# openai/whisper

Measured on AMD Instinct MI355X. Metric: audio-seconds transcribed per wall-second (large-v3 greedy), higher is better.
Workload: dtype f16

## Files before the change

whisper_amd/csrc/gemv.hip:

```cpp
#include "common.h"
#include "kernels.h"
#include <stdlib.h>

#ifndef WH_GEMV8_MAX_ROWS
#define WH_GEMV8_MAX_ROWS 24
#endif

namespace {

#define ISSUE_FENCE() asm volatile("" ::: "memory")

constexpr int CS = 4;

__device__ __forceinline__ float4v load_part4(const float* p) { return *(const float4v*)p; }
__device__ __forceinline__ float4v load_part4(const half_t* p) {
  const half4v h = *(const half4v*)p;
  return float4v{(float)h[0], (float)h[1], (float)h[2], (float)h[3]};
}

template <typename T> struct Pack4;
template <> struct Pack4<float> {
  static __device__ __forceinline__ void store(float* p, float a, float b, float c, float d) {
    *(float4v*)p = float4v{a, b, c, d};
  }
// ... 856 lines not shown
    }
    const bool diag = (lane >> 5) == ((lane >> 3) & 1);
#pragma unroll
    for (int rt = 0; rt < NRT; ++rt) {
      float4v acc = {0.f, 0.f, 0.f, 0.f};
      if constexpr (XW != 0) {
        half8v xt[NU];
#pragma unroll
        for (int u = 0; u < NU; ++u) xt[u] = xfrag[rt * FRAG + (kw * NU + u) * 64 + lane];
#pragma unroll
        for (int u = 0; u < NU; ++u) acc = __builtin_amdgcn_mfma_f32_16x16x32_f16(wa[u], xt[u], acc, 0, 0, 0);
      } else {
#pragma unroll
        for (int u = 0; u < NU; ++u) acc = __builtin_amdgcn_mfma_f32_16x16x32_f16(wa[u], xb[rt][u], acc, 0, 0, 0);
      }
#pragma unroll
      for (int e = 0; e < 4; ++e) {
        float z = diag ? acc[e] : 0.f;
        z += lane_xor8(z);
        float p, q; lane_swap32(z, p, q);
        acc[e] = p + q;
      }
      if (lane < 32 && (lane & 15) < 8) {
#pragma unroll
        for (int e = 0; e < 4; ++e) red[mw][rt][4 * (lane >> 4) + e][lane & 7] = acc[e];
      }
    }
  }
  WH_PROBE_AT(a, wgid, 4);
  __syncthreads();
  WH_PROBE_AT(a, wgid, 5);
#pragma unroll
  for (int j = 0; j < NOUT; ++j) {
    const int o = tid + NT * j;
    const int es = o / (NRT * 64), ert = (o >> 6) % NRT, er = (o >> 3) & 7, ej = o & 7;
    const int en = blockIdx.x * fw + es * 8 + ej;
    const bool on = o < GS * NRT * 64 && ert * 8 + er < R && es * 8 + ej < fw && en < a.N;
    if (on) {
      float v = e_bias[j];
#pragma unroll
      for (int k = 0; k < KS; ++k) v += red[es * KS + k][ert][ej][er];
      const int64_t rr = r0 + ert * 8 + er;
      const int n = en;
      switch (a.epi) {
        case whk::EPI_STORE: ((half_t*)a.y)[a.y_frag ? frag_elem(rr, n, a.N) : rr * a.y_ld + n] = (half_t)v; break;
        case whk::EPI_GELU: ((half_t*)a.y)[a.y_frag ? frag_elem(rr, n, a.N) : rr * a.y_ld + n] = (half_t)gelu_erf(v); break;
        case whk::EPI_F32: ((float*)a.y)[rr * a.y_ld + n] = v; break;
        case whk::EPI_RESID: a.resid[rr * a.resid_ld + n] = e_res[j] + v; break;
        case whk::EPI_QKV: {
          const int D = a.D;
          if (n < D) ((half_t*)a.y)[rr * a.y_ld + n] = (half_t)v;
          else {
            const int64_t pos = e_pos - e_lag[j];
            if (n < 2 * D) ((half_t*)a.kcache)[rr * a.cache_bs + pos * D + (n - D)] = (half_t)v;
            else ((half_t*)a.vcache)[rr * a.cache_bs + pos * D + (n - 2 * D)] = (half_t)v;
          }
        } break;
      }
    }
  }
  WH_PROBE_AT(a, wgid, 6);
  if (a.bump && blockIdx.x == 0 && blockIdx.y == 0 && tid == 0) atomicAdd(a.bump, a.bump_by);
  if (a.bump2 && blockIdx.x == 0 && blockIdx.y == 0 && tid == 0) atomicAdd(a.bump2, 1);
}

template <int PRO, int GS, int KS, int CSm, int XW, int NRT>
hipError_t launch_gemv8_nrt(const whk::GemvArgs& a, int fw, hipStream_t stream) {
  constexpr int WAVES = GS * KS + XW;
  static_assert(WAVES <= 16, "at most 1024 threads per workgroup");
  if (fw < 1 || fw > 8 * GS) return hipErrorInvalidValue;
  whk::g_form = WH_FORM_NAME("gemv8/%s/gs%d/ks%d/xw%d/rt%d", PRO == whk::PRO_PLAIN ? "plain" : PRO == whk::PRO_LN ? "LN" :
                             CSm == 2 ? "combine2" : CSm == 3 ? "combine3" : "combine4", GS, KS, XW, NRT);
  const int nblk = a.K / 64;
  const int nu = (nblk + KS - 1) / KS;
  dim3 grid((a.N + fw - 1) / fw, (a.R + 8 * NRT - 1) / (8 * NRT)), block(WAVES * 64);
  if constexpr (KS == 2) {
    if (nu > 10) return hipErrorInvalidValue;
    hipLaunchKernelGGL((gemv8_kernel<PRO, GS, KS, 10, CSm, XW, NRT>), grid, block, 0, stream, a, fw);
  } else {
    if (nu <= 3) hipLaunchKernelGGL((gemv8_kernel<PRO, GS, KS, 3, CSm, XW, NRT>), grid, block, 0, stream, a, fw);
    else if (nu <= 5) hipLaunchKernelGGL((gemv8_kernel<PRO, GS, KS, 5, CSm, XW, NRT>), grid, block, 0, stream, a, fw);
    else return hipErrorInvalidValue;
  }
  return hipGetLastError();
}

template <int PRO, int GS, int KS, int CSm, int XW>
hipError_t launch_gemv8_cfg(const whk::GemvArgs& a, int fw, hipStream_t stream) {
  if (a.R <= 8) return launch_gemv8_nrt<PRO, GS, KS, CSm, XW, 1>(a, fw, stream);
  if (a.R <= 16) return launch_gemv8_nrt<PRO, GS, KS, CSm, XW, 2>(a, fw, stream);
  if constexpr (GS * KS + XW < 16) {
    if (a.R > 24) return launch_gemv8_nrt<PRO, GS, KS, CSm, XW, 6>(a, fw, stream);
  }
  return launch_gemv8_nrt<PRO, GS, KS, CSm, XW, 3>(a, fw, stream);
}

static int gemv8_fw(int N, int gs) {
  static int ncu = 256;
  int fw = (N + ncu - 1) / ncu;
  if (fw > 8 * gs) fw = 8 * gs;
  if (fw < 4) fw = N < 8 ? N : 8 < 8 * gs ? 8 : 8 * gs;
  return fw;
}

static int gemv8_slots(int N, int pro) {
  const int ngroups = (N + 7) / 8;
  if (pro == whk::PRO_LN) return ngroups >= 600 ? 3 : ngroups >= 400 ? 2 : 1;
  return 1;
}

template <int PRO, int CSm>
hipError_t launch_gemv8_pro(const whk::GemvArgs& a, hipStream_t stream) {
  const int nblk = a.K / 64, gs = gemv8_slots(a.N, PRO), fw = gemv8_fw(a.N, gs);
  if constexpr (PRO == whk::PRO_PLAIN) {
    if (nblk > 20) {
      whk::GemvArgs b = a;
      b.w_ordered = !WH_DEV_FLAG("WH_GEMV8_W_OPERAND_ORDER");
      return launch_gemv8_cfg<PRO, 1, 16, CSm, 0>(b, fw, stream);
    }
    return launch_gemv8_cfg<PRO, 1, 4, CSm, 0>(a, fw, stream);
  } else {
    if constexpr (PRO == whk::PRO_LN) {
      if (gs == 3 && a.R > 8 && !WH_DEV_FLAG("WH_GEMV8_LN3_KS4")) {
        if (a.R <= 16) return launch_gemv8_nrt<PRO, 3, 2, CSm, 8, 2>(a, fw, stream);
        return launch_gemv8_nrt<PRO, 3, 2, CSm, 8, 3>(a, fw, stream);
      }
      if (gs == 3) return launch_gemv8_cfg<PRO, 3, 4, CSm, 4>(a, fw, stream);
      if (gs == 2) return launch_gemv8_cfg<PRO, 2, 4, CSm, 8>(a, fw, stream);
    }
    return launch_gemv8_cfg<PRO, 1, 4, CSm, 8>(a, fw, stream);
  }
}

bool gemv8_applies(const whk::GemvArgs& a) {
  if (WH_DEV_FLAG("WH_GEMV_DOT2")) return false;
  if (a.variant != 0 || a.R < 1 || a.R > 96 || a.K % 64 != 0) return false;
  const int nblk = a.K / 64;
  if (nblk > 20 && (a.pro != whk::PRO_PLAIN || (nblk + 15) / 16 > 5)) return false;
  if (a.epi == whk::EPI_F32 && a.N > 16384) return false;
  if ((int64_t)a.N * a.K >= (1ll << 31)) return false;
  switch (a.pro) {
    case whk::PRO_PLAIN: return a.x_ld % 8 == 0 && (int64_t)a.R * a.x_ld < (1ll << 30);
    case whk::PRO_LN: return a.ln_folded && a.xf_ld % 4 == 0 && (int64_t)a.R * a.xf_ld < (1ll << 29);
    case whk::PRO_COMBINE:
      return a.K == a.H * 64 && a.H <= 20 && a.splits >= 2 && a.splits <= 4 && (int64_t)a.R * a.H * a.splits * 64 < (1ll << 29);
  }
  return false;
}

hipError_t launch_gemv8(const whk::GemvArgs& a, hipStream_t stream) {
  if (a.pro == whk::PRO_PLAIN) return launch_gemv8_pro<whk::PRO_PLAIN, 1>(a, stream);
  if (a.pro == whk::PRO_LN) return launch_gemv8_pro<whk::PRO_LN, 1>(a, stream);
  if (a.pro == whk::PRO_COMBINE && a.splits == 2) return launch_gemv8_pro<whk::PRO_COMBINE, 2>(a, stream);
  if (a.pro == whk::PRO_COMBINE && a.splits == 3) return launch_gemv8_pro<whk::PRO_COMBINE, 3>(a, stream);
  if (a.pro == whk::PRO_COMBINE && a.splits == 4) return launch_gemv8_pro<whk::PRO_COMBINE, 4>(a, stream);
  return hipErrorInvalidValue;
}

template <int NFT>
__global__ __launch_bounds__(1024) void gemv_rows48_kernel(whk::GemvArgs a) {
  extern __shared__ __attribute__((aligned(16))) char smem[];
  pin_kernargs(a);
  constexpr int WAVES = 16, RT = 48, KSP = WAVES / NFT, J = 5, NU = (40 + KSP - 1) / KSP;
  const int K = a.K, nks = K / 32;
  half_t* xs = (half_t*)smem;
  float* red = (float*)smem;
  const int tid = threadIdx.x, lane = tid & 63;
  const int wave = __builtin_amdgcn_readfirstlane(tid >> 6);
  const int ft = wave % NFT, ksp = wave / NFT;
  const int i16 = lane & 15, g4 = lane >> 4;
  const int n0 = blockIdx.x * (NFT * 16);
  const int R = a.R;

  float4v v[3][J];
#pragma unroll
  for (int i = 0; i < 3; ++i) {
    const int r = wave + WAVES * i;
    const float* src = a.xf + (int64_t)(r < R ? r : 0) * a.xf_ld;
#pragma unroll
    for (int j = 0; j < J; ++j) {
      int k = (j * 64 + lane) * 4; if (k > K - 4) k = K - 4;
      v[i][j] = *(const float4v*)(src + k);
    }
  }
  ISSUE_FENCE();
  half8v w[NU];
  {
    int n = n0 + ft * 16 + i16; if (n > a.N - 1) n = a.N - 1;
    const half_t* base = (const half_t*)a.W + (int64_t)n * K + g4 * 8;
#pragma unroll
    for (int u = 0; u < NU; ++u) {
      int st = ksp + KSP * u; if (st > nks - 1) st = nks - 1;
      w[u] = __builtin_nontemporal_load((const half8v*)(base + st * 32));
    }
  }
  ISSUE_FENCE();
  int e_pos = 0;
  if (a.epi == whk::EPI_QKV) e_pos = load_agent_int(a.d_pos);
  float e_bias[(NFT * 768 + 1023) / 1024];
#pragma unroll
  for (int q = 0; q < (NFT * 768 + 1023) / 1024; ++q) {
    const int o = tid + q * 1024;
    int n = n0 + ((o >> 8) / 3) * 16 + (o & 15); if (n > a.N - 1) n = a.N - 1;
    e_bias[q] = a.bias ? a.bias[n] : 0.f;
  }

  {
    const float invK = 1.0f / (float)K;
#pragma unroll
    for (int i = 0; i < 3; ++i) {
      const int r = wave + WAVES * i;
      float sum = 0.f;
#pragma unroll
      for (int j = 0; j < J; ++j) {
        const float t = (v[i][j][0] + v[i][j][1]) + (v[i][j][2] + v[i][j][3]);
        sum += ((j * 64 + lane) * 4 < K) ? t : 0.f;
      }
      const float mean = wave_sum(sum) * invK;
      float ss = 0.f;
#pragma unroll
      for (int j = 0; j < J; ++j) {
        if ((j * 64 + lane) * 4 < K) {
#pragma unroll
          for (int e = 0; e < 4; ++e) { const float d = v[i][j][e] - mean; ss = __builtin_fmaf(d, d, ss); }
        }
      }
      const float rstd = r < R ? rsqrtf(wave_sum(ss) * invK + 1e-5f) : 0.f;
      half_t* xr = xs + (size_t)r * K;
#pragma unroll
      for (int j = 0; j < J; ++j) {
        const int k = (j * 64 + lane) * 4;
        if (k < K)
          Pack4<half_t>::store(xr + ((((k >> 3) ^ (r & 15)) << 3) | (k & 7)), (v[i][j][0] - mean) * rstd,
                               (v[i][j][1] - mean) * rstd, (v[i][j][2] - mean) * rstd, (v[i][j][3] - mean) * rstd);
      }
    }
  }
  __syncthreads();

  float4v acc[3];
#pragma unroll
  for (int rt = 0; rt < 3; ++rt) acc[rt] = float4v{0.f, 0.f, 0.f, 0.f};
#pragma unroll
  for (int u = 0; u < NU; ++u) {
    const int st = ksp + KSP * u;
    if (st < nks) {
#pragma unroll
      for (int rt = 0; rt < 3; ++rt) {
        const half8v xf = *(const half8v*)(xs + (size_t)(rt * 16 + i16) * K + (((st * 4 + g4) ^ i16) << 3));
        acc[rt] = __builtin_amdgcn_mfma_f32_16x16x32_f16(w[u], xf, acc[rt], 0, 0, 0);
      }
    }
  }
  __syncthreads();
#pragma unroll
  for (int rt = 0; rt < 3; ++rt) *(float4v*)(red + ((((ksp * NFT + ft) * 3 + rt) * 16 + i16) * 16 + g4 * 4)) = acc[rt];
  __syncthreads();

#pragma unroll
  for (int q = 0; q < (NFT * 768 + 1023) / 1024; ++q) {
    const int o = tid + q * 1024;
    if (o >= NFT * 768) continue;
    const int f = o & 15, j = (o >> 4) & 15, rt = (o >> 8) % 3, oft = (o >> 8) / 3;
    const int row = rt * 16 + j, n = n0 + oft * 16 + f;
    if (row >= R || n >= a.N) continue;
    float val = e_bias[q];
#pragma unroll
    for (int k = 0; k < KSP; ++k) val += red[((((k * NFT + oft) * 3 + rt) * 16 + j) * 16) + f];
    const int64_t rr = row;
    switch (a.epi) {
      case whk::EPI_STORE: ((half_t*)a.y)[rr * a.y_ld + n] = (half_t)val; break;
      case whk::EPI_GELU: ((half_t*)a.y)[rr * a.y_ld + n] = (half_t)gelu_erf(val); break;
      case whk::EPI_QKV: {
        const int D = a.D;
        if (n < D) ((half_t*)a.y)[rr * a.y_ld + n] = (half_t)val;
        else {
          const int64_t pos = e_pos - (a.lag ? a.lag[row] : 0);
          if (n < 2 * D) ((half_t*)a.kcache)[rr * a.cache_bs + pos * D + (n - D)] = (half_t)val;
          else ((half_t*)a.vcache)[rr * a.cache_bs + pos * D + (n - 2 * D)] = (half_t)val;
        }
      } break;
      default: break;
    }
  }
  if (a.bump && blockIdx.x == 0 && tid == 0) atomicAdd(a.bump, a.bump_by);
  if (a.bump2 && blockIdx.x == 0 && tid == 0) atomicAdd(a.bump2, 1);
}

bool rows48_applies(const whk::GemvArgs& a) {
  return !WH_DEV_FLAG("WH_NO_ROWS48") && a.R > WH_GEMV8_MAX_ROWS && a.R <= 48 && a.pro == whk::PRO_LN && a.ln_folded &&
         a.K % 256 == 0 && a.K <= 1280 && a.N >= 2048 && a.variant <= 0 &&
         (a.epi == whk::EPI_STORE || a.epi == whk::EPI_GELU || a.epi == whk::EPI_QKV);
}

hipError_t launch_rows48(const whk::GemvArgs& a, hipStream_t stream) {
  whk::g_form = "rows48";
  const size_t lds = (size_t)48 * a.K * 2 > 49152 ? (size_t)48 * a.K * 2 : 49152;
  static whk::LdsAttr attr2;
  { hipError_t e = whk::raise_dynamic_lds(attr2, (const void*)gemv_rows48_kernel<2>, 160 * 1024); if (e != hipSuccess) return e; }
  hipLaunchKernelGGL((gemv_rows48_kernel<2>), dim3((a.N + 31) / 32), dim3(1024), lds, stream, a);
  return hipGetLastError();
}

__global__ __launch_bounds__(1024) void gemv_rows48_stream_kernel(whk::GemvArgs a) {
  extern __shared__ __attribute__((aligned(16))) char smem[];
  pin_kernargs(a);
  constexpr int WAVES = 16, J = 5, NB = 20;
  const int K = a.K, nks = K / 32;
  half_t* xs = (half_t*)smem;
  float* gb = (float*)(smem + (size_t)48 * K * 2);
  const int tid = threadIdx.x, lane = tid & 63;
  const int wave = __builtin_amdgcn_readfirstlane(tid >> 6);
  const int i16 = lane & 15, g4 = lane >> 4;
  const int R = a.R;
  const int ntiles = (a.N + 15) / 16;

  float4v v[3][J];
#pragma unroll
  for (int i = 0; i < 3; ++i) {
    const int r = wave + WAVES * i;
    const float* src = a.xf + (int64_t)(r < R ? r : 0) * a.xf_ld;
#pragma unroll
    for (int j = 0; j < J; ++j) {
      int k = (j * 64 + lane) * 4; if (k > K - 4) k = K - 4;
      v[i][j] = *(const float4v*)(src + k);
    }
  }
  for (int k = tid * 4; k < K; k += 4096) {
    *(float4v*)(gb + k) = *(const float4v*)(a.ln_w + k);
    *(float4v*)(gb + K + k) = *(const float4v*)(a.ln_b + k);
  }
  __syncthreads();
  {
    const float invK = 1.0f / (float)K;
#pragma unroll
    for (int i = 0; i < 3; ++i) {
      const int r = wave + WAVES * i;
      float sum = 0.f;
#pragma unroll
      for (int j = 0; j < J; ++j) {
        const float t = (v[i][j][0] + v[i][j][1]) + (v[i][j][2] + v[i][j][3]);
        sum += ((j * 64 + lane) * 4 < K) ? t : 0.f;
      }
      const float mean = wave_sum(sum) * invK;
      float ss = 0.f;
#pragma unroll
      for (int j = 0; j < J; ++j) {
        if ((j * 64 + lane) * 4 < K) {
#pragma unroll
          for (int e = 0; e < 4; ++e) { const float d = v[i][j][e] - mean; ss = __builtin_fmaf(d, d, ss); }
        }
      }
      const float rstd = rsqrtf(wave_sum(ss) * invK + 1e-5f);
      half_t* xr = xs + (size_t)r * K;
#pragma unroll
      for (int j = 0; j < J; ++j) {
        const int k = (j * 64 + lane) * 4;
        if (k < K) {
          const float4v w4 = *(const float4v*)(gb + k), b4 = *(const float4v*)(gb + K + k);
          half_t* dst = xr + ((((k >> 3) ^ (r & 15)) << 3) | (k & 7));
          if (r < R)
            Pack4<half_t>::store(dst, (v[i][j][0] - mean) * rstd * w4[0] + b4[0], (v[i][j][1] - mean) * rstd * w4[1] + b4[1],
                                 (v[i][j][2] - mean) * rstd * w4[2] + b4[2], (v[i][j][3] - mean) * rstd * w4[3] + b4[3]);
          else
            Pack4<half_t>::store(dst, 0.f, 0.f, 0.f, 0.f);
        }
      }
    }
  }
  __syncthreads();

  for (int tile = blockIdx.x * WAVES + wave; tile < ntiles; tile += gridDim.x * WAVES) {
    int n = tile * 16 + i16; if (n > a.N - 1) n = a.N - 1;
    const half_t* base = (const half_t*)a.W + (int64_t)n * K + g4 * 8;
    float4v acc[3];
#pragma unroll
    for (int rt = 0; rt < 3; ++rt) acc[rt] = float4v{0.f, 0.f, 0.f, 0.f};
    for (int st0 = 0; st0 < nks; st0 += NB) {
      half8v w[NB];
#pragma unroll
      for (int u = 0; u < NB; ++u) {
        int st = st0 + u; if (st > nks - 1) st = nks - 1;
        w[u] = __builtin_nontemporal_load((const half8v*)(base + st * 32));
      }
#pragma unroll
      for (int u = 0; u < NB; ++u) {
        const int st = st0 + u;
        if (st < nks) {
#pragma unroll
          for (int rt = 0; rt < 3; ++rt) {
            const half8v xf = *(const half8v*)(xs + (size_t)(rt * 16 + i16) * K + (((st * 4 + g4) ^ i16) << 3));
            acc[rt] = __builtin_amdgcn_mfma_f32_16x16x32_f16(w[u], xf, acc[rt], 0, 0, 0);
          }
        }
      }
    }
#pragma unroll
    for (int rt = 0; rt < 3; ++rt) {
      const int row = rt * 16 + i16;
      if (row < R) {
        float* y = (float*)a.y + (int64_t)row * a.y_ld + tile * 16 + g4 * 4;
#pragma unroll
        for (int e = 0; e < 4; ++e)
          if (tile * 16 + g4 * 4 + e < a.N) y[e] = acc[rt][e];
      }
    }
  }
  if (a.bump && blockIdx.x == 0 && tid == 0) atomicAdd(a.bump, a.bump_by);
  if (a.bump2 && blockIdx.x == 0 && tid == 0) atomicAdd(a.bump2, 1);
}

bool rows48_stream_applies(const whk::GemvArgs& a) {
  return !WH_DEV_FLAG("WH_NO_ROWS48") && a.R > 16 && a.R <= 48 && a.pro == whk::PRO_LN && a.epi == whk::EPI_F32 && !a.bias &&
         a.K % 256 == 0 && a.K <= 1280 && a.N >= 16384 && a.variant <= 0;
}

hipError_t launch_rows48_stream(const whk::GemvArgs& a, hipStream_t stream) {
  whk::g_form = "rows48_stream";
  const size_t lds = (size_t)48 * a.K * 2 + (size_t)2 * a.K * 4;
  static whk::LdsAttr attr;
  { hipError_t e = whk::raise_dynamic_lds(attr, (const void*)gemv_rows48_stream_kernel, 160 * 1024); if (e != hipSuccess) return e; }
  const int ntiles = (a.N + 15) / 16;
  int wgs = (ntiles + 15) / 16;
  if (wgs > 256) wgs = 256;
  hipLaunchKernelGGL(gemv_rows48_stream_kernel, dim3(wgs), dim3(1024), lds, stream, a);
  return hipGetLastError();
}

template <typename T, int MS>
__global__ __launch_bounds__(256) void merge_partials_kernel(const T* __restrict__ part_o, const float* __restrict__ part_ml,
                                                             int S, int R, int H, T* __restrict__ out, int64_t o_ld, int o_frag) {
  const int i = blockIdx.x * 256 + threadIdx.x;
  if (i >= R * H * 16) return;
  const int r = i / (H * 16), rem = i - r * (H * 16);
  const int h = rem >> 4, d4 = rem & 15;
  const int64_t pb = (int64_t)r * H + h, ps = (int64_t)R * H;
  float2v ml[MS];
  float4v o[MS];
#pragma unroll
  for (int s = 0; s < MS; ++s) {
    const int sc = s < S ? s : S - 1;
    ml[s] = *(const float2v*)(part_ml + (pb + sc * ps) * 2);
    o[s] = load_part4(part_o + (pb + sc * ps) * 64 + d4 * 4);
  }
  float M = WH_NEG_INF;
#pragma unroll
  for (int s = 0; s < MS; ++s) { if (s >= S) ml[s] = float2v{WH_NEG_INF, 0.f}; M = fmaxf(M, ml[s][0]); }
  float w[MS], den = 0.f;
#pragma unroll
  for (int s = 0; s < MS; ++s) {
    w[s] = (ml[s][0] == WH_NEG_INF) ? 0.f : __expf(ml[s][0] - M);
    den = __builtin_fmaf(w[s], ml[s][1], den);
  }
  const float inv = 1.0f / den;
  float4v num = {0.f, 0.f, 0.f, 0.f};
#pragma unroll
  for (int s = 0; s < MS; ++s) {
    const float f = w[s] * ml[s][1] * inv;
    num[0] = __builtin_fmaf(f, o[s][0], num[0]); num[1] = __builtin_fmaf(f, o[s][1], num[1]);
    num[2] = __builtin_fmaf(f, o[s][2], num[2]); num[3] = __builtin_fmaf(f, o[s][3], num[3]);
  }
  Pack4<T>::store(out + (o_frag ? frag_elem(r, h * 64 + d4 * 4, H * 64) : (int64_t)r * o_ld + h * 64 + d4 * 4), num[0], num[1], num[2], num[3]);
}

enum class Family { refuse, gemv8, rows48, rows48_stream, rows16_mf, rt4, rt8 };

Family pick_family(const whk::GemvArgs& a, int dtype) {
  if (a.R <= 0) return Family::refuse;
  if (a.x_frag || a.y_frag) return dtype == 1 && a.R <= WH_GEMV8_MAX_ROWS && gemv8_applies(a) ? Family::gemv8 : Family::refuse;
  if (dtype != 1) return a.R <= 4 || a.K > 3072 ? Family::rt4 : Family::rt8;
  if (rows48_applies(a)) return Family::rows48;
  if (rows48_stream_applies(a)) return Family::rows48_stream;
  const bool rows16 = a.R > 8 && a.variant <= 0 && a.K % 128 == 0 && a.K <= 5120 && (a.K / 32 <= 40 || a.pro == whk::PRO_PLAIN);
  if ((a.R <= WH_GEMV8_MAX_ROWS || !rows16) && gemv8_applies(a)) return Family::gemv8;
  if (a.R <= 4) return Family::rt4;
  if (rows16) return Family::rows16_mf;
  return Family::rt8;
}

}

namespace whk {

thread_local const char* g_form = "";

hipError_t launch_gemv(const GemvArgs& a, int dtype, hipStream_t stream) {
  const Family f = pick_family(a, dtype);
  if (dtype == 1) {
    switch (f) {
      case Family::gemv8: return launch_gemv8(a, stream);
      case Family::rows48: return launch_rows48(a, stream);
      case Family::rows48_stream: return launch_rows48_stream(a, stream);
      case Family::rt4: return launch_rt<half_t, 4>(a, stream);
      case Family::rows16_mf: return launch_rows16_mf<half_t>(a, stream);
      case Family::rt8: return launch_rt<half_t, 8>(a, stream);
      case Family::refuse: break;
    }
  } else if (f == Family::rt4 || f == Family::rt8) {
    return f == Family::rt4 ? launch_rt<float, 4>(a, stream) : launch_rt<float, 8>(a, stream);
  }
  return hipErrorInvalidValue;
}

const char* gemv_family(const GemvArgs& a, int dtype) {
  static const char* const names[] = {"", "gemv8", "rows48", "rows48_stream", "rows16_mf", "rt4", "rt8"};
  return names[(int)pick_family(a, dtype)];
}

bool gemv8_will_run(int R, int N, int K, int pro) {
  GemvArgs a = {};
  a.pro = pro; a.R = R; a.N = N; a.K = K; a.x_ld = a.xf_ld = K; a.ln_folded = 1; a.splits = 2; a.H = K / 64;
  a.epi = EPI_STORE; a.y_frag = 1;
  return pick_family(a, 1) == Family::gemv8;
}

hipError_t launch_merge_partials(const void* part_o, const float* part_ml, int splits, int R, int H, void* out,
                                 int64_t o_ld, int dtype, hipStream_t stream, int o_frag) {
  if (splits < 1 || splits > DEC_ATTN_MAX_SPLITS || R <= 0 || H <= 0) return hipErrorInvalidValue;
  const int n = R * H * 16;
  const dim3 grid((n + 255) / 256), block(256);
  g_form = dtype == 1 ? (splits <= 4 ? "merge<half,4>" : "merge<half,16>") : (splits <= 4 ? "merge<float,4>" : "merge<float,16>");
  if (dtype == 1) {
    if (splits <= 4)
      hipLaunchKernelGGL((merge_partials_kernel<half_t, 4>), grid, block, 0, stream, (const half_t*)part_o, part_ml, splits, R, H, (half_t*)out, o_ld, o_frag);
    else
      hipLaunchKernelGGL((merge_partials_kernel<half_t, DEC_ATTN_MAX_SPLITS>), grid, block, 0, stream, (const half_t*)part_o, part_ml, splits, R, H, (half_t*)out, o_ld, o_frag);
  } else {
    if (splits <= 4)
      hipLaunchKernelGGL((merge_partials_kernel<float, 4>), grid, block, 0, stream, (const float*)part_o, part_ml, splits, R, H, (float*)out, o_ld, o_frag);
    else
      hipLaunchKernelGGL((merge_partials_kernel<float, DEC_ATTN_MAX_SPLITS>), grid, block, 0, stream, (const float*)part_o, part_ml, splits, R, H, (float*)out, o_ld, o_frag);
  }
  return hipGetLastError();
}

}
```

Measured before the change: 1164.

## Double-buffer weight streaming in rows48 stream GEMV with LDS transpose and RT templating

Rewrites the LN-fused logits GEMV stream kernel so each wave keeps two register batches of weight loads in flight. While one batch is consumed, the next is prefetched, and the first batch is issued before the LayerNorm prologue to hide its latency. Weights are loaded as contiguous 64-element row segments and transposed through a per-wave LDS scratch area for coalescing. Row tiles are templated (2 or 3) so small batches skip a third of the MFMAs, and the grid now launches up to 256 blocks with tiles interleaved across blocks. This adds LDS traffic and register pressure and needs nks to be divisible by 8.

```diff
diff --git a/whisper_amd/csrc/gemv.hip b/whisper_amd/csrc/gemv.hip
--- a/whisper_amd/csrc/gemv.hip
+++ b/whisper_amd/csrc/gemv.hip
@@ -1182,39 +1182,61 @@
   return hipGetLastError();
 }
 
+template <int RT>
 __global__ __launch_bounds__(1024) void gemv_rows48_stream_kernel(whk::GemvArgs a) {
   extern __shared__ __attribute__((aligned(16))) char smem[];
   pin_kernargs(a);
-  constexpr int WAVES = 16, J = 5, NB = 20;
+  constexpr int WAVES = 16, J = 5, NB = 8;
   const int K = a.K, nks = K / 32;
+  const int nb = nks / NB;
   half_t* xs = (half_t*)smem;
-  float* gb = (float*)(smem + (size_t)48 * K * 2);
+  float* gb = (float*)(smem + (size_t)(16 * RT) * K * 2);
   const int tid = threadIdx.x, lane = tid & 63;
   const int wave = __builtin_amdgcn_readfirstlane(tid >> 6);
   const int i16 = lane & 15, g4 = lane >> 4;
+  half8v* turn = (half8v*)gb + wave * 128;
   const int R = a.R;
   const int ntiles = (a.N + 15) / 16;
-
-  float4v v[3][J];
-#pragma unroll
-  for (int i = 0; i < 3; ++i) {
-    const int r = wave + WAVES * i;
-    const float* src = a.xf + (int64_t)(r < R ? r : 0) * a.xf_ld;
-#pragma unroll
-    for (int j = 0; j < J; ++j) {
-      int k = (j * 64 + lane) * 4; if (k > K - 4) k = K - 4;
-      v[i][j] = *(const float4v*)(src + k);
-    }
-  }
-  for (int k = tid * 4; k < K; k += 4096) {
-    *(float4v*)(gb + k) = *(const float4v*)(a.ln_w + k);
-    *(float4v*)(gb + K + k) = *(const float4v*)(a.ln_b + k);
-  }
-  __syncthreads();
+  const int tstride = gridDim.x * WAVES;
+  const int t0 = blockIdx.x + gridDim.x * wave;
+  const int T = t0 < ntiles ? ((ntiles - t0 + tstride - 1) / tstride) * nb : 0;
+
+  auto load_batch = [&](int tile, int b, half8v* w) {
+#pragma unroll
+    for (int u = 0; u < NB; ++u) {
+      int n = tile * 16 + (u & 1) * 8 + (lane >> 3); if (n > a.N - 1) n = a.N - 1;
+      const int kb = b * (NB / 2) + (u >> 1);
+      w[u] = __builtin_nontemporal_load((const half8v*)((const half_t*)a.W + (int64_t)n * K + kb * 64 + (lane & 7) * 8));
+    }
+  };
+  half8v wa[NB], wb[NB];
+  int lt = T > 0 ? t0 : (int)blockIdx.x, lb = 0;
+
   {
+    float4v v[RT][J];
+#pragma unroll
+    for (int i = 0; i < RT; ++i) {
+      const int r = wave + WAVES * i;
+      const float* src = a.xf + (int64_t)(r < R ? r : 0) * a.xf_ld;
+#pragma unroll
+      for (int j = 0; j < J; ++j) {
+        int k = (j * 64 + lane) * 4; if (k > K - 4) k = K - 4;
+        v[i][j] = *(const float4v*)(src + k);
+      }
+    }
+    int kg = tid * 4; if (kg > K - 4) kg = K - 4;
+    const float4v gw = *(const float4v*)(a.ln_w + kg), gv = *(const float4v*)(a.ln_b + kg);
+    ISSUE_FENCE();
+    load_batch(lt, 0, wa);
+    ISSUE_FENCE();
+    if (tid * 4 < K) {
+      *(float4v*)(gb + kg) = gw;
+      *(float4v*)(gb + K + kg) = gv;
+    }
+    __syncthreads();
     const float invK = 1.0f / (float)K;
 #pragma unroll
-    for (int i = 0; i < 3; ++i) {
+    for (int i = 0; i < RT; ++i) {
       const int r = wave + WAVES * i;
       float sum = 0.f;
 #pragma unroll
@@ -1248,43 +1270,56 @@
       }
     }
   }
+  if (T > 1 && ++lb == nb) { lb = 0; lt += tstride; }
+  ISSUE_FENCE();
+  load_batch(lt, lb, wb);
+  ISSUE_FENCE();
+  if (++lb == nb) { lb = 0; lt += tstride; }
   __syncthreads();
 
-  for (int tile = blockIdx.x * WAVES + wave; tile < ntiles; tile += gridDim.x * WAVES) {
-    int n = tile * 16 + i16; if (n > a.N - 1) n = a.N - 1;
-    const half_t* base = (const half_t*)a.W + (int64_t)n * K + g4 * 8;
-    float4v acc[3];
-#pragma unroll
-    for (int rt = 0; rt < 3; ++rt) acc[rt] = float4v{0.f, 0.f, 0.f, 0.f};
-    for (int st0 = 0; st0 < nks; st0 += NB) {
-      half8v w[NB];
-#pragma unroll
-      for (int u = 0; u < NB; ++u) {
-        int st = st0 + u; if (st > nks - 1) st = nks - 1;
-        w[u] = __builtin_nontemporal_load((const half8v*)(base + st * 32));
-      }
-#pragma unroll
-      for (int u = 0; u < NB; ++u) {
-        const int st = st0 + u;
-        if (st < nks) {
-#pragma unroll
-          for (int rt = 0; rt < 3; ++rt) {
-            const half8v xf = *(const half8v*)(xs + (size_t)(rt * 16 + i16) * K + (((st * 4 + g4) ^ i16) << 3));
-            acc[rt] = __builtin_amdgcn_mfma_f32_16x16x32_f16(w[u], xf, acc[rt], 0, 0, 0);
-          }
-        }
-      }
-    }
-#pragma unroll
-    for (int rt = 0; rt < 3; ++rt) {
-      const int row = rt * 16 + i16;
-      if (row < R) {
-        float* y = (float*)a.y + (int64_t)row * a.y_ld + tile * 16 + g4 * 4;
-#pragma unroll
-        for (int e = 0; e < 4; ++e)
-          if (tile * 16 + g4 * 4 + e < a.N) y[e] = acc[rt][e];
-      }
-    }
+  if (T > 0) {
+    int ct = t0, cb = 0;
+    float4v acc[RT];
+#pragma unroll
+    for (int rt = 0; rt < RT; ++rt) acc[rt] = float4v{0.f, 0.f, 0.f, 0.f};
+    const int wr = lane ^ ((lane >> 4) & 7);
+    const int rd = i16 * 8 + (g4 ^ (i16 >> 1));
+    auto consume = [&](const half8v* w) {
+#pragma unroll
+      for (int p = 0; p < NB / 2; ++p) {
+        const int st = cb * NB + 2 * p;
+        turn[wr] = w[2 * p];
+        turn[64 + (wr ^ 4)] = w[2 * p + 1];
+        const half8v f0 = turn[rd], f1 = turn[rd ^ 4];
+#pragma unroll
+        for (int rt = 0; rt < RT; ++rt) {
+          const half_t* xr = xs + (size_t)(rt * 16 + i16) * K;
+          acc[rt] = __builtin_amdgcn_mfma_f32_16x16x32_f16(*(const half8v*)(xr + (((st * 4 + g4) ^ i16) << 3)), f0, acc[rt], 0, 0, 0);
+          acc[rt] = __builtin_amdgcn_mfma_f32_16x16x32_f16(*(const half8v*)(xr + (((st * 4 + 4 + g4) ^ i16) << 3)), f1, acc[rt], 0, 0, 0);
+        }
+      }
+      if (++cb < nb) return;
+      const int n = ct * 16 + i16;
+#pragma unroll
+      for (int rt = 0; rt < RT; ++rt) {
+#pragma unroll
+        for (int e = 0; e < 4; ++e) {
+          const int row = rt * 16 + g4 * 4 + e;
+          if (row < R && n < a.N) ((float*)a.y)[(int64_t)row * a.y_ld + n] = acc[rt][e];
+        }
+        acc[rt] = float4v{0.f, 0.f, 0.f, 0.f};
+      }
+      cb = 0; ct += tstride;
+    };
+    auto prefetch = [&](half8v* w) {
+      load_batch(lt, lb, w);
+      if (++lb == nb) { lb = 0; lt += tstride; }
+    };
+    int q = 0;
+    for (; q + 3 < T; q += 2) { consume(wa); prefetch(wa); consume(wb); prefetch(wb); }
+    consume(wa);
+    if (T - q == 3) { prefetch(wa); consume(wb); consume(wa); }
+    else if (T - q == 2) consume(wb);
   }
   if (a.bump && blockIdx.x == 0 && tid == 0) atomicAdd(a.bump, a.bump_by);
   if (a.bump2 && blockIdx.x == 0 && tid == 0) atomicAdd(a.bump2, 1);
@@ -1295,16 +1330,20 @@
          a.K % 256 == 0 && a.K <= 1280 && a.N >= 16384 && a.variant <= 0;
 }
 
+template <int RT>
+hipError_t launch_rows48_stream_rt(const whk::GemvArgs& a, hipStream_t stream) {
+  const size_t lds = (size_t)(16 * RT) * a.K * 2 + 16 * 2048;
+  static whk::LdsAttr attr;
+  { hipError_t e = whk::raise_dynamic_lds(attr, (const void*)gemv_rows48_stream_kernel<RT>, 160 * 1024); if (e != hipSuccess) return e; }
+  const int ntiles = (a.N + 15) / 16;
+  const int wgs = ntiles < 256 ? ntiles : 256;
+  hipLaunchKernelGGL(gemv_rows48_stream_kernel<RT>, dim3(wgs), dim3(1024), lds, stream, a);
+  return hipGetLastError();
+}
+
 hipError_t launch_rows48_stream(const whk::GemvArgs& a, hipStream_t stream) {
   whk::g_form = "rows48_stream";
-  const size_t lds = (size_t)48 * a.K * 2 + (size_t)2 * a.K * 4;
-  static whk::LdsAttr attr;
-  { hipError_t e = whk::raise_dynamic_lds(attr, (const void*)gemv_rows48_stream_kernel, 160 * 1024); if (e != hipSuccess) return e; }
-  const int ntiles = (a.N + 15) / 16;
-  int wgs = (ntiles + 15) / 16;
-  if (wgs > 256) wgs = 256;
-  hipLaunchKernelGGL(gemv_rows48_stream_kernel, dim3(wgs), dim3(1024), lds, stream, a);
-  return hipGetLastError();
+  return a.R <= 32 ? launch_rows48_stream_rt<2>(a, stream) : launch_rows48_stream_rt<3>(a, stream);
 }
 
 template <typename T, int MS>
```

After: 1163. About the same (-0.1%).
